# mythos-bio/mythos

Hardware: AMD Instinct MI355X
Metric: MD steps/sec (and ns/day) per GPU, oxDNA2 12 kbp duplex (higher is better)
Workload: dtype f32; 1 GPU; oxDNA2 12000 bp duplex (24000 nt), Debye-Hueckel salt 0.5, Langevin dt 0.005, free space, 1 replica/GPU; half_charged_ends=True, replicas=1, repeats=1, warmup_steps_done=10605, precision=headline f32 (north_star: fp32 at 1e-3); the other precision: --full, full=False

## Files before the change

mythos_amd/csrc/langevin_step.h:

```cpp
#pragma once
#include <hip/hip_runtime.h>

#include <cstdint>

#include "oxdna_gather.h"
#include "philox.h"

namespace mythos {

template <typename R>
struct LangevinConst {
  R dt, half_dt;
  R inv_mass;
  R inv_inertia[3];
  R c1_t, c2_t;
  R c1_r, c2_r[3];
  R skin_half_sq;
};

template <int K, typename R>
__device__ __forceinline__ void free_rotor(R* q, R* L, R h, const R* inv_I) {
  const R phi = h * L[K] * inv_I[K];
  R s, c;
  if constexpr (sizeof(R) == 4) {
    s = __sinf(R(0.5) * phi);
    c = __cosf(R(0.5) * phi);
  } else {
    R x = R(0.5) * phi;
    int halvings = 0;
    const bool large = __ballot(fabs(x) >= R(0.03125)) != 0ull;
    if (large)
      while (fabs(x) >= R(0.03125) && halvings < 64) x *= R(0.5), ++halvings;
    const R x2 = x * x;
    s = x * (R(1) + x2 * (R(-1.0 / 6) + x2 * (R(1.0 / 120) + x2 * R(-1.0 / 5040))));
    c = R(1) + x2 * (R(-0.5) + x2 * (R(1.0 / 24) + x2 * R(-1.0 / 720)));
    if (large)
      for (; halvings > 0; --halvings) {
        const R s2 = R(2) * s * c;
        c = c * c - s * s;
        s = s2;
      }
  }
  const R q0 = q[0], q1 = q[1], q2 = q[2], q3 = q[3];
  if constexpr (K == 0) {
    q[0] = c * q0 - s * q1;
    q[1] = c * q1 + s * q0;
    q[2] = c * q2 + s * q3;
    q[3] = c * q3 - s * q2;
  } else if constexpr (K == 1) {
    q[0] = c * q0 - s * q2;
    q[1] = c * q1 - s * q3;
    q[2] = c * q2 + s * q0;
    q[3] = c * q3 + s * q1;
  } else {
    q[0] = c * q0 - s * q3;
    q[1] = c * q1 + s * q2;
    q[2] = c * q2 - s * q1;
    q[3] = c * q3 + s * q0;
  }
  const R cf = c * c - s * s, sf = R(2) * s * c;
  constexpr int A = (K + 1) % 3, B = (K + 2) % 3;
  const R la = L[A], lb = L[B];
  L[A] = cf * la + sf * lb;
  L[B] = -sf * la + cf * lb;
}

template <typename R>
__device__ __forceinline__ void drift(R* x, R* q, const R* p, R* L, R h, const LangevinConst<R>& K) {
  x[0] += h * p[0] * K.inv_mass;
  x[1] += h * p[1] * K.inv_mass;
  x[2] += h * p[2] * K.inv_mass;
  free_rotor<2>(q, L, R(0.5) * h, K.inv_inertia);
  free_rotor<1>(q, L, R(0.5) * h, K.inv_inertia);
  free_rotor<0>(q, L, h, K.inv_inertia);
  free_rotor<1>(q, L, R(0.5) * h, K.inv_inertia);
  free_rotor<2>(q, L, R(0.5) * h, K.inv_inertia);
}

constexpr int kMdBlock = 256;
constexpr int kMdG = 8;
constexpr int kMdPPB = kMdBlock / kMdG;
#ifndef MYTHOS_MD_ITEMS
#define MYTHOS_MD_ITEMS 16
#endif
#ifndef MYTHOS_MD_F64_BLOCKS
#define MYTHOS_MD_F64_BLOCKS 3
#endif
#ifndef MYTHOS_MD_F64S_BLOCKS
#define MYTHOS_MD_F64S_BLOCKS 2
#endif
#ifndef MYTHOS_MD_F32_BLOCKS
#define MYTHOS_MD_F32_BLOCKS 3
#endif
#ifndef MYTHOS_MD_F32S_BLOCKS
#define MYTHOS_MD_F32S_BLOCKS 2
#endif
constexpr int kMdItems = MYTHOS_MD_ITEMS;
template <typename R, bool SAVE>
constexpr int md_items_big() {
  return (sizeof(R) == 8 && SAVE) ? 22 : 32;
}
#ifndef MYTHOS_MD_POOL
#define MYTHOS_MD_POOL 320
#endif
constexpr int kMdPool = MYTHOS_MD_POOL;
constexpr int kTraceWidth = T_COUNT + 2;

template <typename R>
struct Frame {
  typename Vec4T<R>::type *p0, *p1, *p2, *p3, *q, *pl, *mom, *ang;
};

template <typename R>
constexpr bool kHiLo = sizeof(R) == 4;

template <typename R>
__device__ __forceinline__ V3<R> centre_diff(const typename Vec4T<R>::type& o_hi, const typename Vec4T<R>::type& o_lo,
                                             const V3<R>& s_hi, const V3<R>& s_lo) {
  V3<R> d{o_hi.x - s_hi.x, o_hi.y - s_hi.y, o_hi.z - s_hi.z};
  if constexpr (kHiLo<R>) {
    d.x += o_lo.x - s_lo.x;
    d.y += o_lo.y - s_lo.y;
    d.z += o_lo.z - s_lo.z;
  }
  return d;
}

template <typename R>
struct MdCut {
  R rbb2;
  R rcom2;
  R hb_lo2, hb_hi2, cr_lo2, cr_hi2, cx_lo2, cx_hi2;
  unsigned int hb_mask;
};

template <typename R>
__device__ __forceinline__ V3<R> xyz(const typename Vec4T<R>::type& v) {
  return V3<R>{v.x, v.y, v.z};
}

template <typename R>
__device__ __forceinline__ R f3_coef(R eps, R tw, const F3P<R>& fp, R r2, R& coef) {
  coef = R(0);
  if (r2 >= fp.rc * fp.rc) return R(0);
  const R r = m_sqrt(r2);
  const FD<R> v = f3_eval(r, eps, fp);
  coef = tw * v.d / r;
  return v.f;
}

template <typename R>
__device__ __forceinline__ R f3_radial(R eps, R tw, const F3P<R>& fp, V3<R> d, R r2, V3<R>& g) {
  if (r2 >= fp.rc * fp.rc) return R(0);
  const R r = m_sqrt(r2);
  const FD<R> v = f3_eval(r, eps, fp);
  axpy(g, tw * v.d / r, d);
  return v.f;
}

#ifndef MYTHOS_MD_PRIO_MAP
#define MYTHOS_MD_PRIO_MAP 33210
#endif
#if MYTHOS_MD_PRIO_MAP != 0
constexpr int md_prio_digit(int phase) {
  int v = MYTHOS_MD_PRIO_MAP;
  for (int k = 4; k > phase; --k) v /= 10;
  return v % 10;
}
#define MD_PRIO(phase)                                                     \
  do {                                                                     \
    if (prio_on) __builtin_amdgcn_s_setprio(md_prio_digit(phase));        \
  } while (0)
#else
#define MD_PRIO(phase) do { } while (0)
#endif

template <typename R, bool SAVE, int ITEMS, bool DENSE = false, int MODEL = 2, bool PSEQ = false>
constexpr int md_blocks_per_cu() {
  if (DENSE) return 5;
  if (ITEMS > kMdItems) return sizeof(R) == 4 ? (SAVE ? 1 : 2) : 1;
  return sizeof(R) == 4 ? (SAVE ? MYTHOS_MD_F32S_BLOCKS : MYTHOS_MD_F32_BLOCKS) : (SAVE ? MYTHOS_MD_F64S_BLOCKS : MYTHOS_MD_F64_BLOCKS);
}

template <typename R>
struct RadSet {
  F3P<R> f_bb, f_base, f_bkba, f_babk;
  R eps_n, tw_n, tw_dh;
  DebyeP<R> dhp;
  bool half_ends;
  R rbb2, hb_lo2, hb_hi2, cr_lo2, cr_hi2, cx_lo2, cx_hi2;
  unsigned int hb_mask;
};
template <typename R, int MODEL, class PT>
__device__ __forceinline__ RadSet<R> radset_from(const PT& P, const MdCut<R>& cut) {
  RadSet<R> s;
  s.f_bb = f3_params<R>(P, NEXC_BACKBONE_RSTAR), s.f_base = f3_params<R>(P, NEXC_BASE_RSTAR);
  s.f_bkba = f3_params<R>(P, NEXC_BACK_BASE_RSTAR), s.f_babk = f3_params<R>(P, NEXC_BASE_BACK_RSTAR);
  s.eps_n = P[NEXC_EPS];
  s.tw_n = P[TW_NEXC], s.tw_dh = (MODEL >= 2) ? P[TW_DH] : R(0);
  s.half_ends = (MODEL >= 2) && (P[DH_HALF_CHARGED_ENDS] != R(0));
  s.dhp = (MODEL >= 2) ? debye_params<R>(P) : DebyeP<R>{};
  s.rbb2 = cut.rbb2, s.hb_lo2 = cut.hb_lo2, s.hb_hi2 = cut.hb_hi2, s.cr_lo2 = cut.cr_lo2, s.cr_hi2 = cut.cr_hi2;
  s.cx_lo2 = cut.cx_lo2, s.cx_hi2 = cut.cx_hi2, s.hb_mask = cut.hb_mask;
  return s;
}
template <typename R, class PT>
__device__ __forceinline__ MdCut<R> cut_from(const PT& P, R rcom2) {
  MdCut<R> c;
  const R rbb = fmax(P[NEXC_BACKBONE_RC], P[DH_RCUT]);
  c.rbb2 = rbb * rbb, c.rcom2 = rcom2;
  c.hb_lo2 = P[HYDR_RCLOW] * P[HYDR_RCLOW], c.hb_hi2 = P[HYDR_RCHIGH] * P[HYDR_RCHIGH];
  c.cr_lo2 = P[CRST_RCLOW] * P[CRST_RCLOW], c.cr_hi2 = P[CRST_RCHIGH] * P[CRST_RCHIGH];
  c.cx_lo2 = P[CXST_RCLOW] * P[CXST_RCLOW], c.cx_hi2 = P[CXST_RCHIGH] * P[CXST_RCHIGH];
  c.hb_mask = 0u;
#pragma unroll
  for (int k = 0; k < 16; ++k) c.hb_mask |= (P[HYDR_EPS_00 + k] != R(0)) ? (1u << k) : 0u;
  return c;
}
template <typename R>
__device__ __forceinline__ F3P<R> pick3(const F3P<R>& a, const F3P<R>& b, const F3P<R>& c, int k) {
  return {k == 0 ? a.rstar : (k == 1 ? b.rstar : c.rstar), k == 0 ? a.sigma : (k == 1 ? b.sigma : c.sigma),
          k == 0 ? a.b : (k == 1 ? b.b : c.b), k == 0 ? a.rc : (k == 1 ? b.rc : c.rc), a.base};
}
#define MD_PICK3(f) (k == 0 ? a.f : (k == 1 ? b.f : c.f))
template <typename R>
__device__ __forceinline__ RadSet<R> pick3(const RadSet<R>& a, const RadSet<R>& b, const RadSet<R>& c, int k) {
  RadSet<R> s;
  s.f_bb = pick3(a.f_bb, b.f_bb, c.f_bb, k), s.f_base = pick3(a.f_base, b.f_base, c.f_base, k);
  s.f_bkba = pick3(a.f_bkba, b.f_bkba, c.f_bkba, k), s.f_babk = pick3(a.f_babk, b.f_babk, c.f_babk, k);
  s.eps_n = MD_PICK3(eps_n), s.tw_n = MD_PICK3(tw_n), s.tw_dh = MD_PICK3(tw_dh);
  s.dhp = {MD_PICK3(dhp.rcut), MD_PICK3(dhp.rhigh), MD_PICK3(dhp.kappa), MD_PICK3(dhp.prefactor), MD_PICK3(dhp.bsmooth)};
  s.half_ends = a.half_ends;
  s.rbb2 = MD_PICK3(rbb2), s.hb_lo2 = MD_PICK3(hb_lo2), s.hb_hi2 = MD_PICK3(hb_hi2), s.cr_lo2 = MD_PICK3(cr_lo2);
  s.cr_hi2 = MD_PICK3(cr_hi2), s.cx_lo2 = MD_PICK3(cx_lo2), s.cx_hi2 = MD_PICK3(cx_hi2), s.hb_mask = MD_PICK3(hb_mask);
  return s;
}
#undef MD_PICK3

#define MD_RADSET_OF_ENTRY                                                                                         \
  const int md_kind = (MODEL == 4) ? na1_kind(self.rna, meta_of(o0.w).rna) : 0;                                    \
  const RadSet<R> rs_picked = (MODEL == 4) ? pick3(rs0, rs1, rs2, md_kind) : rs0;                                  \
  const RadSet<R>& rs = (MODEL == 4) ? rs_picked : rs0;
__device__ __forceinline__ int na1_kind(int self_rna, int other_rna) { return (self_rna && other_rna) ? 1 : ((self_rna || other_rna) ? 2 : 0); }

struct Meta {
  int seq, is_end, rna;
};
template <typename R>
__device__ __forceinline__ Meta meta_of(R w) {
  const int m = (int)w;
  return Meta{m & 3, (m >> 2) & 1, (m >> 3) & 1};
}
template <typename R>
__device__ __forceinline__ void set_meta(Nuc<R>& nuc, R w) {
  const Meta m = meta_of(w);
  nuc.seq = m.seq, nuc.is_end = m.is_end, nuc.rna = m.rna;
}
template <typename R>
__device__ __forceinline__ Nuc<R> nuc_from_lds(const R* ms) {
  Nuc<R> nuc;
  nuc.c = V3<R>{ms[0], ms[1], ms[2]};
  nuc.a1 = V3<R>{ms[3], ms[4], ms[5]};
  nuc.a3 = V3<R>{ms[6], ms[7], ms[8]};
  nuc.a2 = cross(nuc.a3, nuc.a1);
  return nuc;
}

template <typename R>
struct NbrState {
  typename Vec4T<R>::type n0{}, n3{}, n1{}, nl{};
  __device__ __forceinline__ void fetch(const Frame<R>& in, int j, bool with_a1) {
    n0 = in.p0[j];
    n3 = in.p3[j];
    if (with_a1) n1 = in.p1[j];
    if constexpr (kHiLo<R>) nl = in.pl[j];
  }
};

template <typename R, int MODEL, bool SAVE, int ITEMS, bool PSEQ = false, bool DENSE = false, int GL = kMdG>
__global__ __launch_bounds__(kMdBlock, (md_blocks_per_cu<R, SAVE, ITEMS, DENSE, MODEL, PSEQ>())) void md_step_kernel(
    const R* __restrict__ Pg, const BoxT<R> box, const LangevinConst<R> K, const MdCut<R> cut, int n, const Frame<R> in,
    const Frame<R> out,
    const int* __restrict__ rows, const int* __restrict__ row_len, const int* __restrict__ row_close, int row_stride,
    int extra_bonds, R kick_close, int do_step, uint64_t seed, uint64_t step, const typename Vec4T<R>::type* __restrict__ ref_pos,
    const typename Vec4T<R>::type* __restrict__ ref_off, const typename Vec4T<R>::type* __restrict__ ref_a1,
    int* __restrict__ flags,
    R* __restrict__ traj_c, R* __restrict__ traj_q, double* __restrict__ e_part, const int* __restrict__ chunk_order,
    const int* __restrict__ list_overflow, int k_index, int , int prio_on, const PseqView<R> pseq) {
  using V4 = typename Vec4T<R>::type;
  constexpr int G = GL, PPB = kMdBlock / GL;
  static_assert(GL == 8 || GL == 16, "lanes per nucleotide");
  static_assert(!DENSE || GL == kMdG, "DENSE serves large grids");
  constexpr int RW = (SAVE ? 12 + T_COUNT : 12) + 1;
  constexpr int kSlots = 2 + ITEMS;
  __shared__ int items[2][PPB][ITEMS];
  __shared__ int item_cnt[2][PPB];
  __shared__ int item_pre[4][PPB + 1];
  __shared__ R self_lds[PPB][13];
  __shared__ R rad_lds[PPB][7];
  static_assert(!DENSE || (sizeof(R) == 4 && !SAVE && !PSEQ && ITEMS == kMdItems && MODEL <= 2), "DENSE: see md_blocks_per_cu");
  constexpr bool kPooled = sizeof(R) == 8 || DENSE;
  constexpr int kPool = (ITEMS > kMdItems || !kPooled) ? PPB * kSlots : kMdPool * PPB / kMdPPB;
  static_assert(kPool >= PPB * ROW_BONDED_SLOTS, "the pool holds at least the bonded rows");
  static_assert(ITEMS > ROW_BONDED_SLOTS, "room for the second-bond slots of circular strands");
  __shared__ R res_flat[kPool * RW + (kPooled ? 0 : PPB)];
  __shared__ int row_base[kPooled ? 4 : 1][PPB + 1];
  constexpr int kFixedStride = (kSlots * RW) | 1;
  auto pool_row = [&](int row) -> R* { return res_flat + row * RW; };
  auto fixed_row = [&](int pp, int slot) -> R* { return res_flat + pp * kFixedStride + slot * RW; };
  __shared__ double e_lds[SAVE ? PPB : 1][kTraceWidth];
  using CP = ConstParams<R, PSEQ>;
  const auto make_cp = [&](const R* g) {
    if constexpr (PSEQ) return CP(g, pseq); else return CP(g);
  };
  const CP P = make_cp(Pg);
  const int grp = threadIdx.x / G;
  const int lane = threadIdx.x % G;
  const int n_blocks = (n + PPB - 1) / PPB;
  const int vb = (int)(blockIdx.x & 7) * ((n_blocks + 7) >> 3) + (int)(blockIdx.x >> 3);
  if (vb >= n_blocks) return;
  __shared__ int s_halt;
  int halt_word = 0;
  if (threadIdx.x == 0) {
    const int hw = flags[1], aw = flags[3];
    halt_word = ((hw != 0 && hw <= k_index) ? 1 : 0) | ((aw != 0 && aw <= k_index) ? 1 : 0) |
                (list_overflow ? (list_overflow[0] | list_overflow[1]) : 0);
  }
  const int bid = chunk_order ? chunk_order[vb] : vb;
  const int i = bid * PPB + grp;
  const bool valid = i < n;
  const int ii = valid ? i : n - 1;

  const R g_ba = P[GEO_BASE], g_st = P[GEO_STACK];
  const CP Prna = make_cp(Pg + ((MODEL == 4) ? OXP_COUNT : 0)), Pdrh = make_cp(Pg + ((MODEL == 4) ? 2 * OXP_COUNT : 0));
  const Na1Params<CP> P4{P, Prna, Pdrh};

  Nuc<R> self;
  V3<R> offb_s, self_lo{R(0), R(0), R(0)};
  {
    const V4 s0 = in.p0[ii], s1 = in.p1[ii], s2 = in.p2[ii], s3 = in.p3[ii];
    if constexpr (kHiLo<R>) self_lo = xyz<R>(in.pl[ii]);
    self.c = xyz<R>(s0);
    self.a1 = xyz<R>(s1);
    self.a3 = xyz<R>(s2);
    self.a2 = cross(self.a3, self.a1);
    offb_s = xyz<R>(s3);
    set_meta(self, s0.w);
    if (lane == 0) {
      R* sl = self_lds[grp];
      sl[0] = s0.x, sl[1] = s0.y, sl[2] = s0.z, sl[3] = s1.x, sl[4] = s1.y, sl[5] = s1.z;
      sl[6] = s2.x, sl[7] = s2.y, sl[8] = s2.z, sl[9] = s0.w;
      sl[10] = self_lo.x, sl[11] = self_lo.y, sl[12] = self_lo.z;
    }
  }
  const int* __restrict__ row = rows + (size_t)ii * row_stride;
  const int len = valid ? row_len[ii] : 0;
  const int close_end = min(len, row_close[ii]);

  R e[T_COUNT];
#pragma unroll
  for (int k = 0; k < T_COUNT; ++k) e[k] = R(0);
  V3<R> gbk{R(0), R(0), R(0)}, gba{R(0), R(0), R(0)};

  MD_PRIO(0);
  const RadSet<R> rs0 = (MODEL == 4) ? radset_from<R, 2>(P, cut_from<R>(P, cut.rcom2)) : radset_from<R, MODEL>(P, cut);
  const RadSet<R> rs1 = (MODEL == 4) ? radset_from<R, 2>(Prna, cut_from<R>(Prna, cut.rcom2)) : rs0;
  const RadSet<R> rs2 = (MODEL == 4) ? radset_from<R, 2>(Pdrh, cut_from<R>(Pdrh, cut.rcom2)) : rs0;
  int n_items[2] = {0, 0};
  const int row_room = ITEMS - (extra_bonds ? ROW_BONDED_SLOTS - 2 : 0);
  const int lane64 = threadIdx.x & 63;
  const int gshift = lane64 & ~(G - 1);
  auto row_at = [&](int s, int end) -> int {
    const int v = row[max(min(s, end - 1), 0)];
    return s < end ? v : -1;
  };
  auto row_word = [&](int s) -> int { return row[max(min(s, len - 1), 0)]; };
  auto slot_of_entry = [&](int e) -> int { return e >= 0 ? (e & ROW_INDEX_MASK) : ii; };
  auto backbone_term = [&](const RadSet<R>& rs, const V3<R>& dco, const V3<R>& offb_o, const V4& o0) __attribute__((always_inline)) {
    const V3<R> d = dco + offb_o - offb_s;
    const R r2 = dot(d, d);
    if (r2 < rs.rbb2) {
      const R r = m_sqrt(r2);
      const FD<R> v = f3_eval(r, rs.eps_n, rs.f_bb);
      R dVdr = rs.tw_n * v.d;
      R en = v.f;
      if constexpr (MODEL >= 2) {
        const FD<R> dh = debye_eval(r, rs.dhp);
        R mult = R(1);
        if (rs.half_ends) mult = (self.is_end ? R(0.5) : R(1)) * (meta_of(o0.w).is_end ? R(0.5) : R(1));
        dVdr += rs.tw_dh * mult * dh.d;
        if constexpr (SAVE) e[T_DH] += R(0.5) * mult * dh.f;
      }
      if constexpr (SAVE) e[T_NEXC] += R(0.5) * en;
      axpy(gbk, dVdr / r, d);
    }
  };
  auto far_entry = [&](const NbrState<R>& o) __attribute__((always_inline)) {
    const V4& o0 = o.n0;
    MD_RADSET_OF_ENTRY
    const V3<R> dco = min_image(centre_diff<R>(o0, o.nl, self.c, self_lo), box);
    backbone_term(rs, dco, xyz<R>(o.n3), o0);
  };
  auto close_entry = [&](int entry, const NbrState<R>& o, bool in_close, bool (&flag)[2]) __attribute__((always_inline)) {
    const V4 &o0 = o.n0, &o1 = o.n1;
    const bool role_p = (entry & ROW_ROLE_Q) == 0;
    MD_RADSET_OF_ENTRY
    const bool o_rna = (MODEL == 4) && meta_of(o0.w).rna;
    const R gba_s = (MODEL == 4 && self.rna) ? Prna[GEO_BASE] : g_ba, gba_o = o_rna ? Prna[GEO_BASE] : g_ba;
    const R gst_s = (MODEL == 4 && self.rna) ? Prna[GEO_STACK] : g_st, gst_o = o_rna ? Prna[GEO_STACK] : g_st;
    (void)gst_s, (void)gst_o;
    const V3<R> dco = min_image(centre_diff<R>(o0, o.nl, self.c, self_lo), box);
    const V3<R> offb_o = xyz<R>(o.n3);
    const bool close = in_close && dot(dco, dco) < cut.rcom2;
    backbone_term(rs, dco, offb_o, o0);
    if (close) {
      const V3<R> a1o = xyz<R>(o1);
      R en = R(0);
      {
        V3<R> dA = dco - offb_s;
        axpy(dA, gba_o, a1o);
        V3<R> dB = dco + offb_o;
        axpy(dB, -gba_s, self.a1);
        const R ra2 = dot(dA, dA), rb2 = dot(dB, dB);
        R c1, c2;
        en += f3_coef(rs.eps_n, rs.tw_n, rs.f_bkba, role_p ? ra2 : rb2, c1);
        en += f3_coef(rs.eps_n, rs.tw_n, rs.f_babk, role_p ? rb2 : ra2, c2);
        axpy(gbk, role_p ? c1 : c2, dA);
        axpy(gba, role_p ? c2 : c1, dB);
      }
      const V3<R> da = a1o - self.a1;
      {
        V3<R> d = dco;
        if constexpr (MODEL == 4) {
          axpy(d, gba_o, a1o);
          axpy(d, -gba_s, self.a1);
        } else {
          axpy(d, g_ba, da);
        }
        const R r2 = dot(d, d);
        en += f3_radial(rs.eps_n, rs.tw_n, rs.f_base, d, r2, gba);
        flag[0] = (rs.cr_lo2 < r2) & (r2 < rs.cr_hi2);
        if (!flag[0] & (rs.hb_lo2 < r2) & (r2 < rs.hb_hi2)) {
          const int so = meta_of(o0.w).seq;
          if (PSEQ && (pseq.terms & 2) != 0)
            flag[0] = rs.hb_mask != 0u;
          else
            flag[0] = (rs.hb_mask >> (role_p ? (self.seq * 4 + so) : (so * 4 + self.seq))) & 1u;
        }
      }
      {
        V3<R> d = dco;
        if constexpr (MODEL == 4) {
          axpy(d, gst_o, a1o);
          axpy(d, -gst_s, self.a1);
        } else {
          axpy(d, g_st, da);
        }
        const R r2 = dot(d, d);
        flag[1] = (rs.cx_lo2 < r2) & (r2 < rs.cx_hi2);
      }
      if constexpr (SAVE) e[T_NEXC] += R(0.5) * en;
    }
  };
  auto append_flagged = [&](const bool (&flag)[2], int entry) __attribute__((always_inline)) {
#pragma unroll
    for (int t = 0; t < 2; ++t) {
      const unsigned long long bal = __ballot(flag[t]);
      const unsigned int gm = (unsigned int)(bal >> gshift) & ((1u << G) - 1u);
      if (flag[t]) {
        const int pos = n_items[t] + __popc(gm & ((1u << lane) - 1u));
        if (pos < ITEMS) items[t][grp][pos] = entry;
      }
      n_items[t] += __popc(gm);
    }
  };
  if constexpr (MODEL == 4 || GL != kMdG) {
    {
      int e_cur = -1, e_nxt = -1;
      NbrState<R> nb;
      {
        const int s = ROW_BONDED_SLOTS + lane;
        e_cur = row_at(s, close_end);
        e_nxt = row_at(s + G, close_end);
        nb.fetch(in, slot_of_entry(e_cur), true);
      }
#pragma unroll 1
      for (int s0 = ROW_BONDED_SLOTS; s0 < close_end; s0 += G) {
        const int s = s0 + lane;
        const int entry = e_cur;
        const V4 o0 = nb.n0, o3 = nb.n3, o1 = nb.n1, ol = nb.nl;
        e_cur = e_nxt;
        e_nxt = row_at(s + 2 * G, close_end);
        nb.fetch(in, slot_of_entry(e_cur), true);
        bool flag[2] = {false, false};
        if (entry >= 0) close_entry(entry, NbrState<R>{o0, o3, o1, ol}, true, flag);
        append_flagged(flag, entry);
      }
    }
    MD_PRIO(1);
    {
      int e_cur = -1, e_nxt = -1;
      NbrState<R> nb;
      {
        const int s = close_end + lane;
        e_cur = row_at(s, len);
        e_nxt = row_at(s + G, len);
        nb.fetch(in, slot_of_entry(e_cur), false);
      }
#pragma unroll 1
      for (int s0 = close_end; s0 < len; s0 += G) {
        const int s = s0 + lane;
        const int entry = e_cur;
        const V4 o0 = nb.n0, o3 = nb.n3, o1 = nb.n1, ol = nb.nl;
        e_cur = e_nxt;
        e_nxt = row_at(s + 2 * G, len);
        nb.fetch(in, slot_of_entry(e_cur), false);
        if (entry >= 0) far_entry(NbrState<R>{o0, o3, o1, ol});
      }
    }
  } else {
    {
      int e_cur = -1, e_nxt = -1;
      NbrState<R> nb;
      int wlen = 0, wclose = 0;
#pragma unroll
      for (int k = 0; k < 64 / G; ++k) {
        wlen = max(wlen, __builtin_amdgcn_readlane(len, k * G));
        wclose = max(wclose, __builtin_amdgcn_readlane(close_end, k * G));
      }
      int s0 = ROW_BONDED_SLOTS;
      if (s0 < wlen) {
        const int s = s0 + lane;
        e_cur = row_at(s, len);
        if (s0 + G < wlen) e_nxt = row_word(s + G);
        nb.fetch(in, slot_of_entry(e_cur), s0 < wclose);
      }
#pragma unroll 1
      for (; s0 < wlen; s0 += G) {
        const int s = s0 + lane;
        const int entry = e_cur;
        const V4 o0 = nb.n0, o3 = nb.n3, o1 = nb.n1, ol = nb.nl;
        e_cur = s + G < len ? e_nxt : -1;
        if (s0 + G < wlen) {
          if (s0 + 2 * G < wlen) e_nxt = row_word(s + 2 * G);
          nb.fetch(in, slot_of_entry(e_cur), s0 + G < wclose);
        }
        if (s0 < wclose) {
          bool flag[2] = {false, false};
          if (entry >= 0) close_entry(entry, NbrState<R>{o0, o3, o1, ol}, s < close_end, flag);
          append_flagged(flag, entry);
        } else {
          MD_PRIO(1);
          if (entry >= 0) far_entry(NbrState<R>{o0, o3, o1, ol});
        }
      }
    }
  }
  if (n_items[0] + n_items[1] > row_room) {
    if (lane == 0) atomicMax(flags + 3, k_index + 1);
    n_items[0] = n_items[1] = 0;
  }
  group_reduce_v3<G>(gbk);
  group_reduce_v3<G>(gba);
  if (lane == 0) {
    R* rl = rad_lds[grp];
    rl[0] = gbk.x, rl[1] = gbk.y, rl[2] = gbk.z, rl[3] = gba.x, rl[4] = gba.y, rl[5] = gba.z;
#pragma unroll
    for (int t = 0; t < 2; ++t) item_cnt[t][grp] = valid ? n_items[t] : 0;
  }
  if (threadIdx.x == 0) s_halt = halt_word;
  __syncthreads();
  MD_PRIO(2);
  if (s_halt != 0) return;
  if (vb == 0 && threadIdx.x == 0) flags[2] = k_index + 1;

  {
    NoPG pg;
    const int wave = ((threadIdx.x >> 6) + bid) & 3;
    const bool bonded_wave = wave == 0;
    const int lst = wave == 3 ? 1 : 0;
    const int pw = threadIdx.x >> 6;
    const int n_bonded_rows = extra_bonds ? ROW_BONDED_SLOTS : 2;
    {
      const int l = threadIdx.x & 63;
      int inc = (l < PPB) ? item_cnt[lst][l] : 0;
      int rows_inc = (kPooled && l < PPB) ? n_bonded_rows + item_cnt[0][l] + item_cnt[1][l] : 0;
#pragma unroll
      for (int o = 1; o < PPB; o <<= 1) {
        const int u = __shfl_up(inc, o, 64);
        if (l >= o) inc += u;
        if constexpr (kPooled) {
          const int v = __shfl_up(rows_inc, o, 64);
          if (l >= o) rows_inc += v;
        }
      }
      if (l < PPB) item_pre[pw][l + 1] = inc;
      if (l == 0) item_pre[pw][0] = 0;
      if constexpr (kPooled) {
        if (l < PPB) row_base[pw][l + 1] = rows_inc;
        if (l == 0) row_base[pw][0] = 0;
      }
      __builtin_amdgcn_wave_barrier();
      __builtin_amdgcn_fence(__ATOMIC_ACQ_REL, "wavefront");
    }
    const bool pool_over = kPooled && row_base[kPooled ? pw : 0][PPB] > kPool;
    if (pool_over && threadIdx.x == 0) atomicMax(flags + 3, k_index + 1);
    const int n_list = pool_over ? 0 : item_pre[pw][PPB];
    const int half = (n_list + 1) >> 1;
    const int q_lo = wave == 2 ? half : 0;
    const int q_hi = wave == 1 ? half : n_list;
    const int n_total = q_hi - q_lo;
    const int n_sweeps = (n_total + 63) / 64;
    const int my_sweeps = bonded_wave ? (pool_over ? 0 : (extra_bonds ? 2 : 1)) : n_sweeps;
    for (int sweep = 0; sweep < my_sweeps; ++sweep) {
      int p, idx, sl;
      bool active;
      if (bonded_wave) {
        p = (threadIdx.x & 63) >> 1;
        idx = (threadIdx.x & 1) + 2 * sweep;
        sl = idx;
        active = p < PPB;
      } else {
        const int q = q_lo + sweep * 64 + (threadIdx.x & 63);
        active = q < q_hi;
        int lo = 0, hi = PPB;
        while (hi - lo > 1) {
          const int mid = (lo + hi) >> 1;
          if (item_pre[pw][mid] <= q) lo = mid; else hi = mid;
        }
        p = lo;
        const int k = q - item_pre[pw][lo];
        sl = active ? items[lst][p][k] : -1;
        idx = n_bonded_rows + k + (lst >= 1 ? item_cnt[0][p] : 0);
      }
      const int ip = bid * PPB + p;
      if (!active || ip >= n) continue;
      const int entry = bonded_wave ? rows[(size_t)ip * row_stride + sl] : sl;
      R* out_r = kPooled ? pool_row(row_base[kPooled ? pw : 0][p] + idx) : fixed_row(p, idx);
      SelfGrad<R> g;
      g.dc = g.g1 = g.g2 = g.g3 = V3<R>{R(0), R(0), R(0)};
      R ee[T_COUNT];
#pragma unroll
      for (int k = 0; k < T_COUNT; ++k) ee[k] = R(0);
      if (entry >= 0) {
        const int j = entry & ROW_INDEX_MASK;
        const bool role_p = bonded_wave ? ((sl & 1) == 1) : ((entry & ROW_ROLE_Q) == 0);
        const R* ms = self_lds[p];
        Nuc<R> me = nuc_from_lds(ms), o;
        set_meta(me, ms[9]);
        me.idx = ip, o.idx = j;
        const V4 o0 = in.p0[j], o1 = in.p1[j], o2 = in.p2[j];
        V4 ol{};
        if constexpr (kHiLo<R>) ol = in.pl[j];
        o.c = xyz<R>(o0);
        o.a1 = xyz<R>(o1);
        o.a3 = xyz<R>(o2);
        o.a2 = cross(o.a3, o.a1);
        set_meta(o, o0.w);
        const V3<R> dco = min_image(centre_diff<R>(o0, ol, me.c, V3<R>{ms[10], ms[11], ms[12]}), box);
        const auto& PP = [&]() -> const auto& {
          if constexpr (MODEL == 4) return P4; else return P;
        }();
        if (wave == 0) {
          bonded_pair<R, MODEL, true, NoPG>(PP, me, o, dco, role_p, R(0.5), ee, g, pg);
        } else if (wave != 3) {
          unbonded_angular<R, MODEL, true, NoPG, 3>(PP, me, o, dco, role_p, R(0.5), ee, g, pg);
        } else {
          unbonded_angular<R, MODEL, true, NoPG, 4>(PP, me, o, dco, role_p, R(0.5), ee, g, pg);
        }
      }
      out_r[0] = g.dc.x, out_r[1] = g.dc.y, out_r[2] = g.dc.z;
      out_r[3] = g.g1.x, out_r[4] = g.g1.y, out_r[5] = g.g1.z;
      out_r[6] = g.g2.x, out_r[7] = g.g2.y, out_r[8] = g.g2.z;
      out_r[9] = g.g3.x, out_r[10] = g.g3.y, out_r[11] = g.g3.z;
      if constexpr (SAVE) {
#pragma unroll
        for (int k = 0; k < T_COUNT; ++k) out_r[12 + k] = ee[k];
      }
    }
  }
  const int int_wave = (3 - bid) & 3;
  const int il = threadIdx.x & 63;
  const int i_int = bid * PPB + il;
  const bool integrates = (int)(threadIdx.x >> 6) == int_wave && il < PPB && i_int < n;
  R z[6] = {R(0), R(0), R(0), R(0), R(0), R(0)};
  V4 pm{}, lm{}, qv{}, r0{}, f0{}, a0{};
  if (integrates) {
    pm = in.mom[i_int], lm = in.ang[i_int], qv = in.q[i_int];
    if (do_step && K.skin_half_sq > R(0)) r0 = ref_pos[i_int], f0 = ref_off[i_int], a0 = ref_a1[i_int];
    if (do_step) normals6(seed, (uint32_t)i_int, step, 0u, z);
#pragma unroll
    for (int k = 0; k < 6; ++k) pin_vgpr(z[k]);
    pin_vgpr(pm.x), pin_vgpr(pm.y), pin_vgpr(pm.z);
    pin_vgpr(lm.x), pin_vgpr(lm.y), pin_vgpr(lm.z);
    pin_vgpr(qv.x), pin_vgpr(qv.y), pin_vgpr(qv.z), pin_vgpr(qv.w);
  }
  __syncthreads();
  MD_PRIO(3);

  SelfGrad<R> sg;
  sg.dc = sg.g1 = sg.g2 = sg.g3 = V3<R>{R(0), R(0), R(0)};
  const int fw = kPooled ? (int)(threadIdx.x >> 6) : 0;
  const int rb = kPooled ? row_base[fw][grp] : 0;
  const bool pool_ok = !kPooled || row_base[fw][PPB] <= kPool;
  const int n_bonded_fold = extra_bonds ? ROW_BONDED_SLOTS : 2;
  if (valid && pool_ok) {
    const int total = kPooled ? row_base[fw][grp + 1] - rb : n_bonded_fold + item_cnt[0][grp] + item_cnt[1][grp];
    for (int u = lane; u < total; u += G) {
      const R* rr = kPooled ? pool_row(rb + u) : fixed_row(grp, u);
      sg.dc = sg.dc + V3<R>{rr[0], rr[1], rr[2]};
      sg.g1 = sg.g1 + V3<R>{rr[3], rr[4], rr[5]};
      sg.g2 = sg.g2 + V3<R>{rr[6], rr[7], rr[8]};
      sg.g3 = sg.g3 + V3<R>{rr[9], rr[10], rr[11]};
      if constexpr (SAVE) {
#pragma unroll
        for (int k = 0; k < T_COUNT; ++k) e[k] += rr[12 + k];
      }
    }
  }
  if (lane == 0) {
    const R* rl = rad_lds[grp];
    const V3<R> rbk{rl[0], rl[1], rl[2]}, rba{rl[3], rl[4], rl[5]};
    sg.dc = sg.dc - (rbk + rba);
    if constexpr (MODEL == 4) {
      const bool r = self.rna != 0;
      axpy(sg.g1, -(r ? Prna[GEO_BACK_A1] : P[GEO_BACK_A1]), rbk);
      axpy(sg.g1, -(r ? Prna[GEO_BASE] : P[GEO_BASE]), rba);
      axpy(sg.g2, r ? R(0) : -P[GEO_BACK_A2], rbk);
      axpy(sg.g3, r ? -Prna[GEO_BACK_A2] : R(0), rbk);
    } else {
    axpy(sg.g1, -P[GEO_BACK_A1], rbk);
    axpy(sg.g1, -P[GEO_BASE], rba);
    if constexpr (MODEL == 2) axpy(sg.g2, -P[GEO_BACK_A2], rbk);
    if constexpr (MODEL == 3) axpy(sg.g3, -P[GEO_BACK_A2], rbk);
    }
  }
  if constexpr (SAVE) {
    group_reduce<G, R, true>(e, sg);
  } else {
    group_reduce_v3<G>(sg.dc);
    group_reduce_v3<G>(sg.g1);
    group_reduce_v3<G>(sg.g2);
    group_reduce_v3<G>(sg.g3);
  }

  if (lane == 0) {
    const Nuc<R> own = nuc_from_lds(self_lds[grp]);
    const V3<R> tl = axes_grad_to_torque(own, sg);
    R* fr = kPooled ? pool_row(pool_ok ? rb : grp * 2) : fixed_row(grp, 0);
    fr[0] = -sg.dc.x, fr[1] = -sg.dc.y, fr[2] = -sg.dc.z;
    fr[3] = dot(own.a1, tl), fr[4] = dot(own.a2, tl), fr[5] = dot(own.a3, tl);
  }
  __syncthreads();
  MD_PRIO(4);
  double ke_t = 0.0, ke_r = 0.0;
  if (integrates) {
    const int i = i_int;
    const Nuc<R> self = nuc_from_lds(self_lds[il]);
    const R* fr = kPooled ? pool_row(row_base[fw][PPB] <= kPool ? row_base[fw][il] : il * 2) : fixed_row(il, 0);
    const V3<R> F{fr[0], fr[1], fr[2]};
    const R tb[3] = {fr[3], fr[4], fr[5]};
    const bool int_rna = (MODEL == 4) && meta_of(self_lds[il][9]).rna;
    const R g_k1 = int_rna ? Prna[GEO_BACK_A1] : P[GEO_BACK_A1];
    const R g_k2 = (MODEL >= 2) ? (int_rna ? Prna[GEO_BACK_A2] : P[GEO_BACK_A2]) : R(0);
    R p[3] = {pm.x, pm.y, pm.z}, L[3] = {lm.x, lm.y, lm.z};
    R qs[4] = {qv.x, qv.y, qv.z, qv.w};
    const R kc = kick_close * K.dt;
    p[0] += kc * F.x;
    p[1] += kc * F.y;
    p[2] += kc * F.z;
    L[0] += kc * tb[0];
    L[1] += kc * tb[1];
    L[2] += kc * tb[2];
    if constexpr (SAVE) {
      ke_t = 0.5 * double(K.inv_mass) * (double(p[0]) * p[0] + double(p[1]) * p[1] + double(p[2]) * p[2]);
      ke_r = 0.5 * (double(K.inv_inertia[0]) * L[0] * L[0] + double(K.inv_inertia[1]) * L[1] * L[1] +
                    double(K.inv_inertia[2]) * L[2] * L[2]);
      if (traj_c) {
        traj_c[3 * i + 0] = self.c.x;
        traj_c[3 * i + 1] = self.c.y;
        traj_c[3 * i + 2] = self.c.z;
      }
      if (traj_q) {
        traj_q[4 * i + 0] = qs[0];
        traj_q[4 * i + 1] = qs[1];
        traj_q[4 * i + 2] = qs[2];
        traj_q[4 * i + 3] = qs[3];
      }
    }
    R x[3] = {self.c.x, self.c.y, self.c.z};
    R xl[3] = {self_lds[il][10], self_lds[il][11], self_lds[il][12]};
    R dxa[3] = {R(0), R(0), R(0)};
    R* const xd = kHiLo<R> ? dxa : x;
    V3<R> n1 = self.a1, n2 = self.a2, n3 = self.a3;
    const bool bk3 = MODEL == 3 || int_rna;
    V3<R> nbk{bk3 ? n3.x : n2.x, bk3 ? n3.y : n2.y, bk3 ? n3.z : n2.z};
    if (do_step) {
      p[0] += K.half_dt * F.x;
      p[1] += K.half_dt * F.y;
      p[2] += K.half_dt * F.z;
      L[0] += K.half_dt * tb[0];
      L[1] += K.half_dt * tb[1];
      L[2] += K.half_dt * tb[2];
      drift(xd, qs, p, L, K.half_dt, K);
      p[0] = K.c1_t * p[0] + K.c2_t * z[0];
      p[1] = K.c1_t * p[1] + K.c2_t * z[1];
      p[2] = K.c1_t * p[2] + K.c2_t * z[2];
      L[0] = K.c1_r * L[0] + K.c2_r[0] * z[3];
      L[1] = K.c1_r * L[1] + K.c2_r[1] * z[4];
      L[2] = K.c1_r * L[2] + K.c2_r[2] * z[5];
      drift(xd, qs, p, L, K.half_dt, K);
      if constexpr (kHiLo<R>) {
#pragma unroll
        for (int k = 0; k < 3; ++k) {
          const R sdl = xl[k] + dxa[k];
          const R t = x[k] + sdl;
          xl[k] = sdl - (t - x[k]);
          x[k] = t;
        }
      }
      const R inv = m_rsqrt(qs[0] * qs[0] + qs[1] * qs[1] + qs[2] * qs[2] + qs[3] * qs[3]);
      qs[0] *= inv;
      qs[1] *= inv;
      qs[2] *= inv;
      qs[3] *= inv;
      if (!(x[0] == x[0]) || !(qs[0] == qs[0])) atomicOr(flags, 2);
      quat_axes(qs[0], qs[1], qs[2], qs[3], n1, n2, n3);
      nbk = V3<R>{bk3 ? n3.x : n2.x, bk3 ? n3.y : n2.y, bk3 ? n3.z : n2.z};
      if (K.skin_half_sq > R(0)) {
        const R dx = x[0] - r0.x, dy = x[1] - r0.y, dz = x[2] - r0.z;
        const R bx = dx + (g_k1 * n1.x + g_k2 * nbk.x - f0.x), by = dy + (g_k1 * n1.y + g_k2 * nbk.y - f0.y),
                bz = dz + (g_k1 * n1.z + g_k2 * nbk.z - f0.z);
        const R gb = int_rna ? Prna[GEO_BASE] : P[GEO_BASE];
        const R sx = dx + gb * (n1.x - a0.x), sy = dy + gb * (n1.y - a0.y), sz = dz + gb * (n1.z - a0.z);
        if (dx * dx + dy * dy + dz * dz > K.skin_half_sq || bx * bx + by * by + bz * bz > K.skin_half_sq ||
            sx * sx + sy * sy + sz * sz > K.skin_half_sq)
          atomicMax(flags + 1, k_index + 1);
      }
    }
    if constexpr (!SAVE) {
      if (traj_c) {
        traj_c[3 * i + 0] = x[0];
        traj_c[3 * i + 1] = x[1];
        traj_c[3 * i + 2] = x[2];
      }
      if (traj_q) reinterpret_cast<V4*>(traj_q)[i] = V4{qs[0], qs[1], qs[2], qs[3]};
    }
    out.p0[i] = V4{x[0], x[1], x[2], self_lds[il][9]};
    if constexpr (kHiLo<R>) out.pl[i] = V4{xl[0], xl[1], xl[2], R(0)};
    out.p1[i] = V4{n1.x, n1.y, n1.z, R(0)};
    out.p2[i] = V4{n3.x, n3.y, n3.z, R(0)};
    out.p3[i] = do_step ? V4{g_k1 * n1.x + g_k2 * nbk.x, g_k1 * n1.y + g_k2 * nbk.y, g_k1 * n1.z + g_k2 * nbk.z, R(0)} : in.p3[i];
    out.q[i] = V4{qs[0], qs[1], qs[2], qs[3]};
    out.mom[i] = V4{p[0], p[1], p[2], R(0)};
    out.ang[i] = V4{L[0], L[1], L[2], R(0)};
  }
  if constexpr (SAVE) {
    if (lane == 0) {
#pragma unroll
      for (int k = 0; k < T_COUNT; ++k) e_lds[grp][k] = valid ? double(e[k]) : 0.0;
    }
    if ((int)(threadIdx.x >> 6) == int_wave && il < PPB) {
      e_lds[il][T_COUNT] = ke_t;
      e_lds[il][T_COUNT + 1] = ke_r;
    }
    __syncthreads();
    if (threadIdx.x < kTraceWidth) {
      double s = 0.0;
      for (int g = 0; g < PPB; ++g) s += e_lds[g][threadIdx.x];
      e_part[(size_t)bid * kTraceWidth + threadIdx.x] = s;
    }
  }
}

}
```

Before: 72150 steps/s.

## Build per-wave interaction lists to replace prefix scan and binary search

For the f32 non-dense DNA path, flagged close pairs are now appended to per-wavefront lists in shared memory, each entry carrying the nucleotide group and slot. The consumer waves find their work by reading four wave counts and indexing directly. This removes the per-group prefix-sum shuffle scan and the binary search over item_pre in the pair-evaluation sweep. A per-wave capacity of 64 adds a new overflow condition that triggers list rebuild.

```diff
diff --git a/mythos_amd/csrc/langevin_step.h b/mythos_amd/csrc/langevin_step.h
--- a/mythos_amd/csrc/langevin_step.h
+++ b/mythos_amd/csrc/langevin_step.h
@@ -293,9 +293,13 @@
   static_assert(!DENSE || GL == kMdG, "DENSE serves large grids");
   constexpr int RW = (SAVE ? 12 + T_COUNT : 12) + 1;
   constexpr int kSlots = 2 + ITEMS;
-  __shared__ int items[2][PPB][ITEMS];
+  constexpr bool kWaveLists = sizeof(R) == 4 && !DENSE && ITEMS == kMdItems && MODEL <= 2 && GL == kMdG;
+  constexpr int kWaveCap = 64;
+  __shared__ int items[kWaveLists ? 1 : 2][kWaveLists ? 1 : PPB][kWaveLists ? 1 : ITEMS];
   __shared__ int item_cnt[2][PPB];
-  __shared__ int item_pre[4][PPB + 1];
+  __shared__ int item_pre[kWaveLists ? 1 : 4][kWaveLists ? 1 : PPB + 1];
+  __shared__ int2 wave_items[kWaveLists ? 2 : 1][kWaveLists ? 4 : 1][kWaveLists ? kWaveCap : 1];
+  __shared__ __attribute__((aligned(16))) int wave_cnt[2][4];
   __shared__ R self_lds[PPB][13];
   __shared__ R rad_lds[PPB][7];
   static_assert(!DENSE || (sizeof(R) == 4 && !SAVE && !PSEQ && ITEMS == kMdItems && MODEL <= 2), "DENSE: see md_blocks_per_cu");
@@ -367,6 +371,8 @@
   const RadSet<R> rs1 = (MODEL == 4) ? radset_from<R, 2>(Prna, cut_from<R>(Prna, cut.rcom2)) : rs0;
   const RadSet<R> rs2 = (MODEL == 4) ? radset_from<R, 2>(Pdrh, cut_from<R>(Pdrh, cut.rcom2)) : rs0;
   int n_items[2] = {0, 0};
+  const int wave_s = __builtin_amdgcn_readfirstlane(threadIdx.x >> 6);
+  int wave_n[2] = {0, 0};
   const int row_room = ITEMS - (extra_bonds ? ROW_BONDED_SLOTS - 2 : 0);
   const int lane64 = threadIdx.x & 63;
   const int gshift = lane64 & ~(G - 1);
@@ -469,9 +475,15 @@
       const unsigned int gm = (unsigned int)(bal >> gshift) & ((1u << G) - 1u);
       if (flag[t]) {
         const int pos = n_items[t] + __popc(gm & ((1u << lane) - 1u));
-        if (pos < ITEMS) items[t][grp][pos] = entry;
+        if constexpr (kWaveLists) {
+          const int wpos = wave_n[t] + (int)__builtin_amdgcn_mbcnt_hi((unsigned)(bal >> 32), __builtin_amdgcn_mbcnt_lo((unsigned)bal, 0u));
+          if (wpos < kWaveCap) wave_items[t][wave_s][wpos] = make_int2(entry, grp | (pos << 8));
+        } else {
+          if (pos < ITEMS) items[t][grp][pos] = entry;
+        }
       }
       n_items[t] += __popc(gm);
+      if constexpr (kWaveLists) wave_n[t] = __builtin_amdgcn_readfirstlane(wave_n[t] + __popcll(bal));
     }
   };
   if constexpr (MODEL == 4 || GL != kMdG) {
@@ -556,9 +568,12 @@
       }
     }
   }
-  if (n_items[0] + n_items[1] > row_room) {
+  bool lists_over = n_items[0] + n_items[1] > row_room;
+  if constexpr (kWaveLists) lists_over = __any(lists_over) || wave_n[0] > kWaveCap || wave_n[1] > kWaveCap;
+  if (lists_over) {
     if (lane == 0) atomicMax(flags + 3, k_index + 1);
     n_items[0] = n_items[1] = 0;
+    wave_n[0] = wave_n[1] = 0;
   }
   group_reduce_v3<G>(gbk);
   group_reduce_v3<G>(gba);
@@ -567,6 +582,9 @@
     rl[0] = gbk.x, rl[1] = gbk.y, rl[2] = gbk.z, rl[3] = gba.x, rl[4] = gba.y, rl[5] = gba.z;
 #pragma unroll
     for (int t = 0; t < 2; ++t) item_cnt[t][grp] = valid ? n_items[t] : 0;
+  }
+  if constexpr (kWaveLists) {
+    if (lane64 == 0) wave_cnt[0][wave_s] = wave_n[0], wave_cnt[1][wave_s] = wave_n[1];
   }
   if (threadIdx.x == 0) s_halt = halt_word;
   __syncthreads();
@@ -581,7 +599,13 @@
     const int lst = wave == 3 ? 1 : 0;
     const int pw = threadIdx.x >> 6;
     const int n_bonded_rows = extra_bonds ? ROW_BONDED_SLOTS : 2;
-    {
+    int wl_b1 = 0, wl_b2 = 0, wl_b3 = 0, wl_n = 0;
+    if constexpr (kWaveLists) {
+      const int4 wc = *reinterpret_cast<const int4*>(wave_cnt[lst]);
+      const int c0 = __builtin_amdgcn_readfirstlane(wc.x), c1 = __builtin_amdgcn_readfirstlane(wc.y);
+      const int c2 = __builtin_amdgcn_readfirstlane(wc.z), c3 = __builtin_amdgcn_readfirstlane(wc.w);
+      wl_b1 = c0, wl_b2 = wl_b1 + c1, wl_b3 = wl_b2 + c2, wl_n = wl_b3 + c3;
+    } else {
       const int l = threadIdx.x & 63;
       int inc = (l < PPB) ? item_cnt[lst][l] : 0;
       int rows_inc = (kPooled && l < PPB) ? n_bonded_rows + item_cnt[0][l] + item_cnt[1][l] : 0;
@@ -605,7 +629,7 @@
     }
     const bool pool_over = kPooled && row_base[kPooled ? pw : 0][PPB] > kPool;
     if (pool_over && threadIdx.x == 0) atomicMax(flags + 3, k_index + 1);
-    const int n_list = pool_over ? 0 : item_pre[pw][PPB];
+    const int n_list = kWaveLists ? wl_n : (pool_over ? 0 : item_pre[kWaveLists ? 0 : pw][kWaveLists ? 0 : PPB]);
     const int half = (n_list + 1) >> 1;
     const int q_lo = wave == 2 ? half : 0;
     const int q_hi = wave == 1 ? half : n_list;
@@ -623,14 +647,23 @@
       } else {
         const int q = q_lo + sweep * 64 + (threadIdx.x & 63);
         active = q < q_hi;
+        int k;
+        if constexpr (kWaveLists) {
+          const int src = (q >= wl_b1) + (q >= wl_b2) + (q >= wl_b3);
+          const int at = q - (q >= wl_b3 ? wl_b3 : q >= wl_b2 ? wl_b2 : q >= wl_b1 ? wl_b1 : 0);
+          const int2 it = wave_items[lst][src][at & (kWaveCap - 1)];
+          p = it.y & (PPB - 1), k = it.y >> 8;
+          sl = active ? it.x : -1;
+        } else {
         int lo = 0, hi = PPB;
         while (hi - lo > 1) {
           const int mid = (lo + hi) >> 1;
           if (item_pre[pw][mid] <= q) lo = mid; else hi = mid;
         }
         p = lo;
-        const int k = q - item_pre[pw][lo];
+        k = q - item_pre[pw][lo];
         sl = active ? items[lst][p][k] : -1;
+        }
         idx = n_bonded_rows + k + (lst >= 1 ? item_cnt[0][p] : 0);
       }
       const int ip = bid * PPB + p;
```

Result: faster. 73900 steps/s, median of 6 (+2.4%).
